# SebLague/Ray-Tracing

Measured on AMD Instinct MI355X. Metric: Mrays/s at 1920x1080, 8 spp, 8 bounces; per-channel L2 vs reference, higher is better.
Workload: dtype f32

## Files before the change

### include/rt_tile_cand.h

```cpp
#ifndef RT_TILE_CAND_ABI_H
#define RT_TILE_CAND_ABI_H

#include "rt_abi.h"

#ifdef __cplusplus
extern "C" {
#endif

int rt_debug_tile_cand(const RtContext* ctx);

#ifdef __cplusplus
}
#endif

#endif
```

### ray-tracing_amd/csrc/rt_context.hip

```cpp
#include <hip/hip_runtime.h>

#include <math.h>
#include <stdarg.h>
#include <stdio.h>
#include <stdlib.h>
#include <string.h>
#include <dlfcn.h>
#include <sys/mman.h>

#include <cmath>
#include <string>
#include <vector>

#include <algorithm>
#include <chrono>
#include <mutex>

#include "rt_kernels.h"
#include "../../include/rt_cost.h"
#include "../../include/rt_primary.h"
#include "../../include/rt_tile_cand.h"
#include "../../include/rt_aov.h"
#include "../../include/rt_denoise.h"
#include "../../include/rt_reproject.h"
// ... 75 lines not shown
    int wavesPerGroup = 1;
    uint32_t hotUnits = 0;
    uint32_t poolSpinLimit = 1u << 16;
    int poolMinItems = 4;
    int poolWaves = 1, poolCells = 0;
    uint32_t travLimit = 1u << 20;
    bool haveScene = false;
    std::vector<RtModel> hModels;
    std::vector<uint32_t> hRootCodes;
    std::vector<int32_t> hTriBase;
    PrimaryTris primaryTris;
    bool primaryOn = true;
    int lastPrimaryOn = -1;
    bool tileCandOn = true;
    int lastTileCand = -1;
    uint32_t* dTileCand[2] = {nullptr, nullptr};
    int tileCandTiles = 0;
    bool tileCandValid[2] = {false, false};
    TileCandKey tileCandKey[2];
    bool tileCandWanted = false;
    TileCandKey tileCandWant;

    RtParams params;
    bool haveParams = false;
    int frame = 1;

    unsigned long long* dCounters = nullptr;
    unsigned long long* dTileQueue = nullptr;
    unsigned long long tileQueueNext[2] = {0, 0};
    uint32_t* dTileCost = nullptr;
// ... 283 lines not shown
        HIP_TRY(ctx, hipStreamSynchronize(ctx->ownStream));
        HIP_TRY(ctx, hipEventCreate(&ctx->evStart));
        HIP_TRY(ctx, hipEventCreate(&ctx->evStop));
        for (hipEvent_t& ev : ctx->backend.ev) HIP_TRY(ctx, hipEventCreateWithFlags(&ev, hipEventDisableTiming));
        return RT_OK;
    };
    if (int rc = init()) {
        rt_destroy(ctx);
        return rc;
    }
    memset(&ctx->params, 0, sizeof(ctx->params));
    if (const char* g = getenv("RT_GRID")) ctx->gridOverride = atoi(g);
    if (const char* g = getenv("RT_POOL_MIN_ITEMS")) ctx->poolMinItems = atoi(g);
    if (const char* g = getenv("RT_PRIMARY")) ctx->primaryOn = atoi(g) != 0;
    if (const char* g = getenv("RT_TILE_CAND")) ctx->tileCandOn = atoi(g) != 0;
    if (const char* g = getenv("RT_POOL_FAULT")) { if (atoi(g)) ctx->poolSpinLimit = 64u | 0x80000000u; }
    if (getenv("RT_VERBOSE")) ctx->verbose = true;
    if (const char* f = getenv("RT_FUSE_FRAMES")) ctx->fuseFrames = atoi(f) != 0;
    if (const char* l = getenv("RT_LPT")) ctx->order.lpt = atoi(l) != 0;
    if (const char* t = getenv("RT_TWO_STREAMS")) ctx->twoStreams = atoi(t) != 0;
    if (const char* c = getenv("RT_COALESCE")) ctx->coalesce = atoi(c) != 0;
    if (const char* fg = getenv("RT_FRAME_GROUP")) ctx->frameGroupOverride = atoi(fg);
    if (const char* al = getenv("RT_ALTERNATE")) ctx->order.alternate = ctx->alternateWanted = atoi(al) != 0;
    ctx->order.set_two_streams(ctx->twoStreams && ctx->sideStream);
    if (const char* fc = getenv("RT_FUSE_CAP"))
        if (const int cap = rt_plan::pinned_fuse_cap(atoi(fc))) { ctx->fuseCap = cap; ctx->fuseCapPinned = true; }
    *out = ctx;
    return RT_OK;
}

// ... 517 lines not shown
        const bool noNegZero = rt_f2u(o.x) != 0x80000000u && rt_f2u(o.y) != 0x80000000u && rt_f2u(o.z) != 0x80000000u;
        a.raygenNoDefocus = (a.defocus == 0.0f && fin && noNegZero && std::isfinite(a.rcpW)) ? 1 : 0;
        const bool allowed = withTable && ctx->haveScene &&
                             primary_allowed(ctx->primaryOn, a.raygenNoDefocus != 0, ctx->flatScene, ctx->nSpheres, ctx->nModels, ctx->primaryTris);
        std::vector<float> sph;
        DModel dm[RT_PRIMARY_MAX_MODELS];
        if (allowed) {
            float bound;
            pack_spheres(ctx->hSpheres.data(), ctx->nSpheres, sph, &bound);
            for (int i = 0; i < ctx->nModels; i++) pack_model(ctx->hModels[i], ctx->hRootCodes[i], ctx->hTriBase[i], dm[i]);
        }
        primary_fill(a.primary, allowed, o, sph.data(), ctx->nSpheres, ctx->sphereBound, dm, ctx->nModels, ctx->primaryTris);
        if (withTable) {
            ctx->lastPrimaryOn = a.primary.on;
            ctx->lastTileCand = 0;
            ctx->tileCandWanted = ctx->tileCandOn && a.primary.on != 0;
            if (ctx->tileCandWanted) {
                TileCandKey& k = ctx->tileCandWant;
                tile_cand_key_init(k);
                memcpy(k.cam, a.cam, sizeof(k.cam));
                memcpy(k.viewParams, a.viewParams, sizeof(k.viewParams));
                k.rcpWm1 = a.rcpWm1; k.rcpHm1 = a.rcpHm1; k.rcpW = a.rcpW; k.diverge = a.diverge;
                k.camOrigin[0] = o.x; k.camOrigin[1] = o.y; k.camOrigin[2] = o.z;
                k.W = (int32_t)a.W; k.H = (int32_t)a.H;
                k.tilesX = a.tilesX; k.tiles = a.tilesX * a.tilesY;
                k.stripRows = a.stripRows; k.partIndex = a.partIndex; k.partCount = a.partCount;
                k.nSpheres = ctx->nSpheres;
                memcpy(k.sph, sph.data(), sizeof(float) * 4 * (size_t)ctx->nSpheres);
            }
        }
    }
    a.counters = ctx->dCounters;
    a.travLimit = ctx->travLimit;
    a.poolSpinLimit = ctx->poolSpinLimit;
    a.wavesPerGroup = 1;
}

}

struct LaunchPlan {
    void (*kern)(const KArgs) = nullptr;
    void (*kernHalf)(const KArgs) = nullptr;
    rt_plan::LaunchShape shape;
// ... 82 lines not shown
    }
    a.tileCost = ctx->dTileCost;
    return RT_OK;
}

static int prepare_tile_cand(RtContext* ctx, int tiles)
{
    if (!ctx->tileCandWanted || ctx->tileCandTiles == tiles) return RT_OK;
    HIP_TRY(ctx, hipStreamSynchronize(joined(ctx)));
    ctx->tileCandTiles = 0;
    for (int s = 0; s < 2; s++) {
        hipFree(ctx->dTileCand[s]); ctx->dTileCand[s] = nullptr;
        ctx->tileCandValid[s] = false;
    }
    for (int s = 0; s < 2; s++)
        if (hipMalloc(&ctx->dTileCand[s], sizeof(uint32_t) * (size_t)tiles) != hipSuccess) {
            (void)hipGetLastError();
            ctx->dTileCand[s] = nullptr;
            ctx->tileCandWanted = false;
            return RT_OK;
        }
    ctx->tileCandTiles = tiles;
    return RT_OK;
}

static_assert(sizeof(float4) == RT_STAGED_PIXEL_BYTES, "a staged colour is one float4");
static int prepare_staging(RtContext* ctx, KArgs& a, int nFrames, size_t nPix, int lane, bool split, bool* unavailable)
{
    *unavailable = false;
    const size_t need = (size_t)nFrames * nPix * RT_STAGED_PIXEL_BYTES;
    if (!ctx->stagingUnavailable && ctx->stagingBytes[lane] < need) {
// ... 159 lines not shown
    hipStream_t st = stream(s);
    a.pxCold = (float4*)((char*)ctx->dPxCold + (size_t)s * ctx->pxColdWaves * RT_COLD_STRIDE_BYTES);
    a.tileQueue = ctx->dTileQueue + s;
    a.tileQueueBase = pp.tileQueueBase;
    a.tileCand = nullptr;
    if (ctx->tileCandWanted && ctx->tileCandTiles == job->tiles && ctx->tileCandWant.tiles == job->tiles) {
        if (!ctx->tileCandValid[s] || memcmp(&ctx->tileCandKey[s], &ctx->tileCandWant, sizeof(TileCandKey)) != 0) {
            ctx->tileCandValid[s] = false;
            hipLaunchKernelGGL(rtk::rt_tile_cand_kernel, dim3((unsigned)((job->tiles + 255) / 256)), dim3(256), 0, st, ctx->tileCandWant, ctx->dTileCand[s]);
            HIP_TRY(ctx, hipGetLastError());
            ctx->tileCandKey[s] = ctx->tileCandWant;
            ctx->tileCandValid[s] = true;
        }
        a.tileCand = ctx->dTileCand[s];
        ctx->lastTileCand = 1;
    }
    RtContext::Tuner::Probe* probe = job->probe;
    const int fuseSlot = nFrames > 1 ? mark_fused_launch_begin(ctx, st) : -1;
    if (probe) hipEventRecord(probe->start, st);
    hipLaunchKernelGGL(parts == 2 ? plan.kernHalf : plan.kern, dim3(pp.grid), dim3(plan.shape.blockThreads), plan.shape.ldsBytes, st, a);
    if (probe) { hipEventRecord(probe->stop, st); probe->live = true; }
    HIP_TRY(ctx, hipGetLastError());
    mark_fused_launch_end(ctx, fuseSlot, st, nFrames);
    ctx->tileQueueNext[s] = pp.queueNext;
    return RT_OK;
}

int HipOrder::accumulate(int s)
{
    int blocks = (int)((job->nPix + 255) / 256);
// ... 291 lines not shown
    if (n > 2 * RT_N_PHASES) out[2 * RT_N_PHASES] = sum_field(h, 6);
    for (int p = 0; p < RT_N_PHASES && 2 * RT_N_PHASES + 1 + p < n; p++) out[2 * RT_N_PHASES + 1 + p] = p < 3 ? sum_field(h, 8 + 2 * RT_N_PHASES + p) : 0;
    return RT_OK;
}

struct DevScratch {
    void* p = nullptr;
    ~DevScratch() { if (p) hipFree(p); }
    hipError_t alloc(size_t bytes) { return hipMalloc(&p, bytes); }
    float* f() const { return (float*)p; }
};

int rt_debug_fused_frames_cap(const RtContext* ctx) { return ctx ? ctx->fuseCap : RT_ERR_INVALID_ARG; }
int rt_debug_primary_table(const RtContext* ctx) { return ctx ? ctx->lastPrimaryOn : RT_ERR_INVALID_ARG; }
int rt_debug_tile_cand(const RtContext* ctx) { return ctx ? ctx->lastTileCand : RT_ERR_INVALID_ARG; }

int rt_debug_intersect(RtContext* ctx, const float* origins, const float* dirs, int n, float* out10)
{
    if (ctx) RT_FLUSH(ctx);
    if (!ctx) return fail(nullptr, RT_ERR_INVALID_ARG, "null context");
    if (!ctx->haveScene) return fail(ctx, RT_ERR_STATE, "rt_debug_intersect before rt_upload_scene");
    if (n < 0 || (n && (!origins || !dirs || !out10))) return fail(ctx, RT_ERR_INVALID_ARG, "rt_debug_intersect: bad arguments");
    if (n == 0) return RT_OK;
    HIP_TRY(ctx, hipSetDevice(ctx->device));
    DevScratch dO, dD, dR;
    HIP_TRY(ctx, dO.alloc((size_t)n * 12));
    HIP_TRY(ctx, dD.alloc((size_t)n * 12));
    HIP_TRY(ctx, dR.alloc((size_t)n * 40));
    HIP_TRY(ctx, hipMemcpy(dO.p, origins, (size_t)n * 12, hipMemcpyHostToDevice));
    HIP_TRY(ctx, hipMemcpy(dD.p, dirs, (size_t)n * 12, hipMemcpyHostToDevice));
// ... 1704 lines not shown
```

### ray-tracing_amd/csrc/rt_kernels.h

```cpp
#ifndef RT_KERNELS_H
#define RT_KERNELS_H

#include <hip/hip_runtime.h>

#include "../../include/rt_abi.h"
#include "../../include/rt_math.h"
#include "rt_device.h"
#include "rt_tile_cand.h"

#ifndef RT_SUSPEND_NUM
#define RT_SUSPEND_NUM 3
#define RT_SUSPEND_DEN 8
#endif
#ifndef RT_INNER_BURST
#define RT_INNER_BURST 3
#endif

namespace rtk {

#define RT_CAS __attribute__((address_space(4)))
#define RT_LDS __attribute__((address_space(3)))

__device__ __forceinline__ float hw_min(float a, float b) { return __builtin_fminf(a, b); }
__device__ __forceinline__ float hw_max(float a, float b) { return __builtin_fmaxf(a, b); }
// ... 145 lines not shown
        bdet = determinant;
    }
}

struct Trav {
    unsigned long long cand;
    int m;
    uint32_t cur;
    int sp;
    bool rootStep;
    rt_f3 lpos, ldir, linv;
    int triBase;
    bool cull;
};

template <bool STATS, bool FLAT, bool MANY, bool ANY = false, bool PRIMARY = false>
__device__ __forceinline__ void begin_intersect(const KArgs& a, rt_f3 rpos, rt_f3 rdir, uint32_t* extBase, SceneHit& h, Trav& t, Stats& st, const float tmax = 0.0f,
                                                const RT_CAS PrimaryTable* pt = nullptr, const uint32_t* tileCand = nullptr, const uint32_t tile = 0u)
{
    h.dst = RT_INF;
    h.obj = -1;
    h.tri = -1;
    h.u = h.v = h.det = 0.0f;
    h.backface = false;

    const RT_CAS float* sph = (const RT_CAS float*)a.spheres;
    const RT_CAS float* sphq = (const RT_CAS float*)a.sphereQuick;
    const float qa = rt_dot(rdir, rdir);
    const float od = __builtin_fmaf(rpos.x, rdir.x, __builtin_fmaf(rpos.y, rdir.y, rpos.z * rdir.z));
    const float oo = PRIMARY ? 0.0f : __builtin_fmaf(rpos.x, rpos.x, __builtin_fmaf(rpos.y, rpos.y, rpos.z * rpos.z));
    const float negMargin = -(7.62939453125e-06f * qa * (PRIMARY ? pt->ooBound : oo + a.sphereBound));
    typedef float rt_f2v __attribute__((ext_vector_type(2)));
    const rt_f2v dx2 = {rdir.x, rdir.x}, dy2 = {rdir.y, rdir.y}, dz2 = {rdir.z, rdir.z};
    const rt_f2v ox2 = {rpos.x, rpos.x}, oy2 = {rpos.y, rpos.y}, oz2 = {rpos.z, rpos.z};
    const rt_f2v od2 = {od, od}, oo2 = {oo, oo}, qa2 = {qa, qa}, m2 = {-2.0f, -2.0f};
    for (int base = 0; base < a.nSpheres; base += 32) {
        const int n = (a.nSpheres - base) < 32 ? (a.nSpheres - base) : 32;
        uint32_t cand = 0;
        if (PRIMARY && tileCand != nullptr) {
            cand = tileCand[tile];
            if (STATS) {
                for (uint32_t rest = ~cand & (n >= 32 ? 0xffffffffu : (1u << n) - 1u); rest; rest &= rest - 1) {
                    const int s = base + __builtin_ctz(rest);
                    const rt_f3 off = rt_v3(pt->sph[s][0], pt->sph[s][1], pt->sph[s][2]);
                    const float qb = 2 * rt_dot(off, rdir);
                    const float disc = qb * qb - 4 * qa * pt->sph[s][3];
                    if (disc >= 0 && (-qb + rt_sqrt(disc)) * rt_rcp(2 * qa) >= 0) st.filterViolations++;
                }
            }
        } else
        for (int k = 0; k < n; k += 2) {
            const RT_CAS float* q = PRIMARY ? &pt->pair[0][0] + 4 * (base + k) : sphq + 4 * (base + k);
            const rt_f2v cx = {q[0], q[1]}, cy = {q[2], q[3]}, cz = {q[4], q[5]}, kk = {q[6], q[7]};
            const rt_f2v cd = __builtin_elementwise_fma(cx, dx2, __builtin_elementwise_fma(cy, dy2, cz * dz2));
            const rt_f2v b = od2 - cd;
            rt_f2v ct = kk;
            if (!PRIMARY) {
                const rt_f2v co = __builtin_elementwise_fma(cx, ox2, __builtin_elementwise_fma(cy, oy2, cz * oz2));
                ct = __builtin_elementwise_fma(m2, co, oo2) + kk;
            }
            const rt_f2v dq = __builtin_elementwise_fma(b, b, -(qa2 * ct));
            const bool keep0 = !(dq.x < negMargin);
            const bool keep1 = (k + 1 < n) && !(dq.y < negMargin);
            if (STATS) {
                for (int j = 0; j < 2 && k + j < n; j++) {
                    const int s = base + k + j;
                    rt_f3 off = rpos - rt_v3(sph[4 * s + 0], sph[4 * s + 1], sph[4 * s + 2]);
                    float qb = 2 * rt_dot(off, rdir);
                    float qc = rt_dot(off, off) - sph[4 * s + 3];
                    float disc = qb * qb - 4 * qa * qc;
                    if (disc >= 0 && !(j ? keep1 : keep0)) st.filterViolations++;
                }
            }
            cand |= ((keep0 ? 1u : 0u) << k) | ((keep1 ? 1u : 0u) << (k + 1));
        }
        if (ANY && h.dst < tmax) cand = 0;
        while (cand) {
            phase_mark<STATS>(st, PH_SPHERE_ROOTS);
            const int k = __builtin_ctz(cand);
            cand &= cand - 1;
            const int s = base + k;
            float4 sp;
            if (PRIMARY) {
                typedef float rt_f4v __attribute__((ext_vector_type(4)));
                const rt_f4v v = *reinterpret_cast<const RT_CAS rt_f4v*>(&pt->sph[s][0]);
                sp = make_float4(v.x, v.y, v.z, v.w);
            }
            else sp = *reinterpret_cast<const float4*>(a.spheres + 4 * s);
            rt_f3 off = PRIMARY ? rt_v3(sp.x, sp.y, sp.z) : rpos - rt_v3(sp.x, sp.y, sp.z);
            float qb = 2 * rt_dot(off, rdir);
            float qc = PRIMARY ? sp.w : rt_dot(off, off) - sp.w;
            float disc = qb * qb - 4 * qa * qc;
            if (!(disc >= 0)) continue;
            float sq = rt_sqrt(disc);
            const float inv2a = rt_rcp(2 * qa);
            float dstNear = rt_max(0.0f, (-qb - sq) * inv2a);
            float dstFar = (-qb + sq) * inv2a;
            if (dstFar >= 0) {
                bool inside = dstNear == 0;
                float d = inside ? dstFar : dstNear;
                if (d < h.dst) {
                    h.dst = d;
                    h.obj = s;
                    h.backface = inside;
                    if (ANY && d < tmax) cand = 0;
                }
            }
        }
    }
    if (STATS) st.sphere += (uint32_t)a.nSpheres;

    unsigned long long cand = 0;
    const RT_CAS DFilter* cf = (const RT_CAS DFilter*)a.filters;
    const int nf = FLAT ? 0 : (MANY ? a.nFiltered : (a.nModels < 64 ? a.nModels : 64));
    if (nf > 0) {
        const rt_f3 winv = rt_v3(__builtin_amdgcn_rcpf(rdir.x), __builtin_amdgcn_rcpf(rdir.y), __builtin_amdgcn_rcpf(rdir.z));
        const bool farOrigin = !(rt_abs(rpos.x) <= a.filterMaxOrigin && rt_abs(rpos.y) <= a.filterMaxOrigin && rt_abs(rpos.z) <= a.filterMaxOrigin);
        auto test_model = [&](int m) -> bool {
            const RT_CAS DFilter& F = cf[m];
            bool keep = true;
// ... 255 lines not shown
                t.cand = 0;
            } else if (t.sp == 0) t.cur = RT_CODE_NEXT_MODEL;
            else t.cur = stackBase[(--t.sp) * RT_WAVE];
        }
        if (++watchdog > a.travLimit) {
            t.cur = RT_CODE_DONE; t.sp = 0; t.cand = 0;
            if ((int)(threadIdx.x & 63) == __ffsll((long long)__ballot(1)) - 1) atomicAdd(a.counters + 7, 1ull);
        }
        RT_TRAV_VOTE();
    } while ((nA + nB + nC) * RT_SUSPEND_DEN > enteredNum);
#undef RT_TRAV_VOTE
    return t.cur == RT_CODE_DONE;
}

template <bool STATS, bool ANY = false, bool PRIMARY = false>
__device__ __forceinline__ void traverse_flat(const KArgs& a, rt_f3 rpos, rt_f3 rdir, SceneHit& h, Stats& st, const float tmax = 0.0f, const RT_CAS PrimaryTable* pt = nullptr)
{
    const RT_CAS DModel* cm = (const RT_CAS DModel*)a.models;
    const DTri* __restrict__ tris = a.tris;
    const RT_CAS float* pr = PRIMARY ? &pt->tri[0][0] : nullptr;
    for (int m = 0; m < a.nModels; m++) {
        if (ANY && __ballot(!(h.dst < tmax)) == 0ull) break;
        const RT_CAS DModel& M = cm[m];
        rt_f3 lpos;
        if (PRIMARY) lpos = rt_v3(pt->lpos[m][0], pt->lpos[m][1], pt->lpos[m][2]);
        else lpos = rt_v3(M.w2l[0] * rpos.x + M.w2l[1] * rpos.y + M.w2l[2] * rpos.z + M.w2l[3] * 1.0f,
                          M.w2l[4] * rpos.x + M.w2l[5] * rpos.y + M.w2l[6] * rpos.z + M.w2l[7] * 1.0f,
                          M.w2l[8] * rpos.x + M.w2l[9] * rpos.y + M.w2l[10] * rpos.z + M.w2l[11] * 1.0f);
        rt_f3 ldir = rt_v3(M.w2l[0] * rdir.x + M.w2l[1] * rdir.y + M.w2l[2] * rdir.z + M.w2l[3] * 0.0f,
                           M.w2l[4] * rdir.x + M.w2l[5] * rdir.y + M.w2l[6] * rdir.z + M.w2l[7] * 0.0f,
                           M.w2l[8] * rdir.x + M.w2l[9] * rdir.y + M.w2l[10] * rdir.z + M.w2l[11] * 0.0f);
        const uint32_t code = M.rootCode;
        uint32_t count = (code >> 24) & 0x7fu;
        uint32_t start = code & RT_CODE_MAX_INLINE_START;
        if (count == 0) {
            count = a.bigLeaves[2 * start + 1];
            start = a.bigLeaves[2 * start];
        }
        if (STATS) { st.leaf++; st.tri += count; }
        const int first = M.triBase + (int)start;
        const bool cull = M.cullBackface != 0;
        for (uint32_t i = 0; i < count; i++) {
            phase_mark<STATS>(st, PH_TRI);
            if (ANY && h.dst < tmax) break;
            const float before = h.dst;
            tri_test<PRIMARY>(tris, first + 3 * (int)i, lpos, ldir, cull, h.dst, h.tri, h.u, h.v, h.det, pr);
            if (PRIMARY) pr += 4;
            if (h.dst < before) {
                h.obj = a.nSpheres + m;
                h.backface = h.det < 0;
            }
        }
    }
}

template <bool STATS>
__device__ __forceinline__ void intersect_scene(const KArgs& a, rt_f3 rpos, rt_f3 rdir, uint32_t* stackBase, uint32_t* extBase, SceneHit& h, Stats& st)
{
    Trav t;
    if (a.nChunks) {
        begin_intersect<STATS, false, true>(a, rpos, rdir, extBase, h, t, st);
        traverse<STATS, false, true>(a, rpos, rdir, stackBase, extBase, h, t, st, (const RT_LDS char*)nullptr, 0u);
    } else {
        begin_intersect<STATS, false, false>(a, rpos, rdir, extBase, h, t, st);
        traverse<STATS, false, false>(a, rpos, rdir, stackBase, extBase, h, t, st, (const RT_LDS char*)nullptr, 0u);
    }
}
// ... 391 lines not shown
                    if constexpr (COST) if (pathActive) {
                        uint4* const o = RT_COST_SLOT(c) + 1;
                        uint4 p = *o;
                        p.x -= st.inner; p.y -= st.leaf; p.z -= st.tri;
                        *o = p;
                    }
                }
            }
            if (pathActive) {
                phase_mark<STATS>(st, PH_SPHERES);
                if constexpr (FLAT && !MANY && !COST) {
                    const RT_CAS PrimaryTable* const pt = &cold_args().primary;
                    if (pt->on != 0 && __ballot(bounce != 0) == 0ull) {
                        const uint32_t* const tileCand = cold_args().tileCand;
                        const uint32_t tile = tileCand ? __float_as_uint(PX_COLD(cold_args())[RT_WAVE].w) : 0u;
                        begin_intersect<STATS, FLAT, MANY, false, true>(a, rpos, rdir, extBase, h, t, st, 0.0f, pt, tileCand, tile);
                        traverse_flat<STATS, false, true>(a, rpos, rdir, h, st, 0.0f, pt);
                    } else {
                        begin_intersect<STATS, FLAT, MANY>(a, rpos, rdir, extBase, h, t, st);
                        traverse_flat<STATS>(a, rpos, rdir, h, st);
                    }
                    segments++;
                    inTrav = true;
                } else {
                    begin_intersect<STATS, FLAT, MANY>(a, rpos, rdir, extBase, h, t, st);
                    segments++;
                    inTrav = true;
                    if (FLAT) traverse_flat<STATS>(a, rpos, rdir, h, st);
                }
            }
        }
        if constexpr (!POOL) {
// ... 347 lines not shown
    __syncthreads();
    if (t == 0) {
        uint32_t run = 0;
        for (int k = 0; k < 1024; k++) { base[k] = run; run += hist[k]; }
    }
    __syncthreads();
    for (int i = t; i < nTiles; i += 1024) order[atomicAdd(&base[key[i]], 1u)] = (uint32_t)i;
}

__global__ void __launch_bounds__(256) rt_tile_cand_kernel(const TileCandKey k, uint32_t* out)
{
    const int tile = (int)(blockIdx.x * 256u + threadIdx.x);
    if (tile >= k.tiles) return;
    int x0, y0;
    tile_cand_origin(k, tile, &x0, &y0);
    out[tile] = tile_cand_mask(k, x0, y0);
}

__global__ void rt_display_kernel(const float4* src, float4* dst, size_t n, int frame)
{
    const float inv = rt_rcp((float)frame);
    size_t i = (size_t)blockIdx.x * blockDim.x + threadIdx.x;
    const size_t stride = (size_t)gridDim.x * blockDim.x;
    for (; i < n; i += stride) {
        float4 v = src[i];
        dst[i] = make_float4(v.x * inv, v.y * inv, v.z * inv, v.w * inv);
    }
}
__global__ void rt_display_srgb8_kernel(const float4* src, uint32_t* dst, int width, int rows, int frame, int flipY)
{
    const float inv = rt_rcp((float)frame);
// ... 53 lines not shown
```

### ray-tracing_amd/csrc/rt_primary.h

```cpp
#ifndef RT_PRIMARY_H
#define RT_PRIMARY_H

#include <math.h>
#include <stdint.h>
#include <string.h>

#include <cmath>

#include "../../include/rt_math.h"
#include "rt_records.h"

#define RT_PRIMARY_MAX_SPHERES 32
#define RT_PRIMARY_MAX_MODELS 4
#define RT_PRIMARY_MAX_TRIS 16

struct alignas(16) PrimaryTable {
    int32_t on;
    float ooBound;
    int32_t pad[2];
    float camOrigin[4];
    float lpos[RT_PRIMARY_MAX_MODELS][4];
    float pair[RT_PRIMARY_MAX_SPHERES / 2][8];
    float sph[RT_PRIMARY_MAX_SPHERES][4];
    float tri[RT_PRIMARY_MAX_TRIS][4];
};

struct PrimaryTris {
    bool usable = false;
    int nModels = 0;
    int count[RT_PRIMARY_MAX_MODELS] = {0, 0, 0, 0};
    float a[RT_PRIMARY_MAX_TRIS][3];
    float face[RT_PRIMARY_MAX_TRIS][3];
};

static inline void primary_collect_tris(bool flat, const DModel* models, int nModels, const unsigned char* triSpace, size_t triSpaceBytes,
                                        const uint32_t* bigLeaves, size_t nBigLeafWords, PrimaryTris& out)
{
    out = PrimaryTris();
    if (!flat || nModels < 0 || nModels > RT_PRIMARY_MAX_MODELS) return;
    int total = 0;
    for (int m = 0; m < nModels; m++) {
        const uint32_t code = models[m].rootCode;
        uint32_t count = (code >> 24) & 0x7fu, start = code & RT_CODE_MAX_INLINE_START;
        if (count == 0) {
            if (2 * (size_t)start + 1 >= nBigLeafWords) return;
            count = bigLeaves[2 * (size_t)start + 1];
            start = bigLeaves[2 * (size_t)start];
        }
        if (count > (uint32_t)(RT_PRIMARY_MAX_TRIS - total)) return;
        for (uint32_t i = 0; i < count; i++) {
            const long long unit = (long long)models[m].triBase + (long long)start + 3ll * (long long)i;
            if (unit < 0 || ((size_t)unit + 3) * 16 > triSpaceBytes) return;
            DTri t;
            memcpy(&t, triSpace + (size_t)unit * 16, sizeof(t));
            out.a[total][0] = t.ax; out.a[total][1] = t.ay; out.a[total][2] = t.az;
            out.face[total][0] = t.fx; out.face[total][1] = t.fy; out.face[total][2] = t.fz;
            total++;
        }
        out.count[m] = (int)count;
    }
    out.nModels = nModels;
    out.usable = true;
}

static inline bool primary_allowed(bool switchOn, bool noDefocus, bool flatScene, int nSpheres, int nModels, const PrimaryTris& tris)
{
    return switchOn && noDefocus && flatScene && nSpheres >= 0 && nSpheres <= RT_PRIMARY_MAX_SPHERES && nModels >= 0 && nModels <= RT_PRIMARY_MAX_MODELS &&
           tris.usable && tris.nModels == nModels;
}

static inline rt_f3 primary_cam_origin(const float* cam) { return rt_mul_point(cam, rt_v3(0.0f, 0.0f, 0.0f), 1.0f); }
// ... 50 lines not shown
```

### ray-tracing_amd/csrc/rt_tile_cand.h

```cpp
#ifndef RT_TILE_CAND_H
#define RT_TILE_CAND_H

#include <stdint.h>
#include <string.h>

#include "../../include/rt_math.h"

#define RT_TILE_CAND_MAX_SPHERES 32

struct TileCandKey {
    float cam[16];
    float viewParams[3];
    float rcpWm1, rcpHm1, rcpW, diverge;
    float camOrigin[3];
    int32_t W, H;
    int32_t tilesX, tiles;
    int32_t stripRows, partIndex, partCount;
    int32_t nSpheres;
    float sph[RT_TILE_CAND_MAX_SPHERES][4];
};

static inline void tile_cand_key_init(TileCandKey& k) { memset(&k, 0, sizeof(k)); }

RT_HD void tile_cand_origin(const TileCandKey& k, int tile, int* x0, int* y0)
{
    const int ty = tile / k.tilesX;
    const int row0 = ty * 8;
    const int ls = row0 / k.stripRows;
    *x0 = (tile - ty * k.tilesX) * 8;
    *y0 = (ls * k.partCount + k.partIndex) * k.stripRows + (row0 - ls * k.stripRows);
}

RT_HD bool tile_cand_finite(float x) { return rt_abs(x) < RT_INF; }

// ... 25 lines not shown
        const float re = slack * rt_sqrt(rr + 7.62939453125e-06f * (D2 + rr)) + scale;
        const float sa2 = slack * slack * (Rt * Rt) / L2, sb2 = slack * slack * (re * re) / D2;
        const rt_f3 cr = rt_cross(a, v);
        const float cross2 = rt_dot(cr, cr), av = rt_dot(a, v);
        const float lim = L2 * D2;
        bool drop = false;
        if (tile_cand_finite(sa2) && tile_cand_finite(sb2) && tile_cand_finite(cross2) && tile_cand_finite(av) && tile_cand_finite(lim) && sa2 + sb2 < 0.98f) {
            const float sg = rt_sqrt(sa2) * rt_sqrt(1.0f - sb2) + rt_sqrt(1.0f - sa2) * rt_sqrt(sb2);
            drop = (av <= 0.0f) || (cross2 > sg * sg * lim);
        }
        if (!drop) mask |= 1u << s;
    }
    return mask;
}

#endif
```

### ray-tracing_amd/hip.py

```python
import ctypes as C
import os

import numpy as np

from . import abi

_HERE = os.path.dirname(os.path.abspath(__file__))
LIB_PATH = os.environ.get("RT_HIP_LIB") or os.path.join(_HERE, "lib", "libraytrace_hip.so")

ABI_SYMBOLS = [
    "rt_create", "rt_destroy", "rt_last_error", "rt_set_stream", "rt_resize", "rt_set_partition", "rt_local_rows",
    "rt_local_to_global_row", "rt_bind_render_targets", "rt_get_render_targets", "rt_upload_scene", "rt_update_models",
    "rt_update_spheres", "rt_set_params", "rt_reset_accumulation", "rt_render_frame", "rt_render_frames",
    "rt_synchronize", "rt_get_frame", "rt_read_frame", "rt_read_accumulated", "rt_display", "rt_display_srgb8",
    "rt_write_accumulated", "rt_timer_begin", "rt_timer_end",
    "rt_enable_stats", "rt_reset_counters", "rt_get_counters", "rt_build_bvh", "rt_build_bvh_mt", "rt_build_bvh_gpu", "rt_build_bvh_gpu_release", "rt_camera_view_params", "rt_version",
    "rt_debug_intersect", "rt_debug_math_eval", "rt_debug_phase_profile", "rt_build_bvh_gpu_batch",
    "rt_flush", "rt_validate_scene", "rt_debug_layout", "rt_debug_layout_free", "rt_debug_fused_frames_cap",
    "rt_create_multi", "rt_destroy_multi", "rt_multi_count", "rt_multi_context", "rt_multi_resize", "rt_multi_upload_scene",
    "rt_multi_update_models", "rt_multi_update_spheres", "rt_multi_set_params", "rt_multi_reset_accumulation",
    "rt_multi_render_frame", "rt_multi_render_frames", "rt_multi_synchronize", "rt_gather_accumulated", "rt_gather_frame",
    "rt_multi_get_counters", "rt_multi_last_gather_ms", "rt_multi_peer_access", "rt_gather_accumulated_to_device", "rt_gather_frame_to_device",
    "rt_gather_rccl",
]
COST_SYMBOLS = ["rt_render_cost"]
PRIMARY_SYMBOLS = ["rt_debug_primary_table"]
TILE_CAND_SYMBOLS = ["rt_debug_tile_cand"]
AOV_SYMBOLS = ["rt_render_aov", "rt_render_aov_to_device"]
DENOISE_SYMBOLS = ["rt_denoise_default_params", "rt_denoise_buffers", "rt_denoise", "rt_denoise_to_device"]
REPROJECT_SYMBOLS = ["rt_reproject_default_params", "rt_reproject_buffers", "rt_reproject_accumulated", "rt_resolve_buffers", "rt_resolve",
                     "rt_resolve_to_device"]
MOTION_SYMBOLS = ["rt_render_aov_centre", "rt_render_aov_centre_to_device", "rt_motion_from_scene", "rt_reproject_buffers_moving",
                  "rt_reproject_accumulated_moving"]
VARIANCE_SYMBOLS = ["rt_denoise_variance_default_params", "rt_moments_update_buffers", "rt_denoise_variance_buffers", "rt_variance_update",
                    "rt_variance_reset", "rt_variance_carry", "rt_variance_read_moments", "rt_variance_moments_to_device", "rt_denoise_variance",
                    "rt_denoise_variance_to_device"]
ADAPTIVE_SYMBOLS = ["rt_adaptive_default_params", "rt_adaptive_select_buffers", "rt_adaptive_select", "rt_adaptive_set_tiles", "rt_adaptive_read_tiles",
                    "rt_adaptive_read_tile_error", "rt_adaptive_render_frames"]
QUERY_SYMBOLS = ["rt_query_closest", "rt_query_closest_buffers", "rt_query_occluded", "rt_query_occluded_buffers"]
RADIANCE_SYMBOLS = ["rt_radiance_trace", "rt_radiance_trace_buffers"]
COST_FIELDS = ("segments", "innerSteps", "leafSteps", "triTests", "primaryInnerSteps", "primaryLeafSteps", "primaryTriTests", "firstHit")

# ... 434 lines not shown
        self._check(self.api.gather_rccl(self.h, nccl_comm, int(root), 1 if accumulated else 0, device_ptr, nbytes))

    def fused_frames_cap(self):
        return self.api.debug_fused_frames_cap(self.h)

    def primary_table(self):
        fn = self.api.lib.rt_debug_primary_table
        fn.restype, fn.argtypes = C.c_int, [C.c_void_p]
        return fn(self.h)

    def tile_cand(self):
        fn = self.api.lib.rt_debug_tile_cand
        fn.restype, fn.argtypes = C.c_int, [C.c_void_p]
        return fn(self.h)

    def synchronize(self):
        self._check(self.api.synchronize(self.h))

    def flush(self):
        self._check(self.api.flush(self.h))

    def timer_begin(self):
        self._check(self.api.timer_begin(self.h))

    def timer_end(self):
        self._check(self.api.timer_end(self.h))

    def enable_stats(self, on=True):
        self._check(self.api.enable_stats(self.h, 1 if on else 0))

# ... 205 lines not shown
```

Baseline: 52920.

## Add per-tile triangle candidate masks to cull primary-ray triangle tests

Extends the per-tile candidate precompute to triangles in flat primary tables. A conservative frustum-versus-triangle-wedge test builds a bitmask per tile, and the wave-wide union of these masks gates which triangles traverse_flat tests for primary rays. When no lane needs any triangle, the flat traversal is skipped entirely. The sphere candidate path is also split out so it no longer runs the 32-sphere base loop. The cost is a doubled candidate buffer, a larger key, ballot/readlane loops, and the risk of wrongly culling a triangle if the conservative bounds are off.

```diff
diff --git a/include/rt_tile_cand.h b/include/rt_tile_cand.h
--- a/include/rt_tile_cand.h
+++ b/include/rt_tile_cand.h
@@ -2,6 +2,7 @@
 #define RT_TILE_CAND_ABI_H
 
 #include "rt_abi.h"
+#include "rt_tile_tri.h"
 
 #ifdef __cplusplus
 extern "C" {
diff --git a/include/rt_tile_tri.h b/include/rt_tile_tri.h
--- /dev/null
+++ b/include/rt_tile_tri.h
@@ -0,0 +1,16 @@
+#ifndef RT_TILE_TRI_ABI_H
+#define RT_TILE_TRI_ABI_H
+
+#include "rt_abi.h"
+
+#ifdef __cplusplus
+extern "C" {
+#endif
+
+int rt_debug_tile_tri(const RtContext* ctx);
+
+#ifdef __cplusplus
+}
+#endif
+
+#endif
diff --git a/ray-tracing_amd/csrc/rt_context.hip b/ray-tracing_amd/csrc/rt_context.hip
--- a/ray-tracing_amd/csrc/rt_context.hip
+++ b/ray-tracing_amd/csrc/rt_context.hip
@@ -113,6 +113,8 @@
     int lastPrimaryOn = -1;
     bool tileCandOn = true;
     int lastTileCand = -1;
+    bool tileTriOn = true;
+    int lastTileTri = -1;
     uint32_t* dTileCand[2] = {nullptr, nullptr};
     int tileCandTiles = 0;
     bool tileCandValid[2] = {false, false};
@@ -426,6 +428,7 @@
     if (const char* g = getenv("RT_POOL_MIN_ITEMS")) ctx->poolMinItems = atoi(g);
     if (const char* g = getenv("RT_PRIMARY")) ctx->primaryOn = atoi(g) != 0;
     if (const char* g = getenv("RT_TILE_CAND")) ctx->tileCandOn = atoi(g) != 0;
+    if (const char* g = getenv("RT_TILE_TRI")) ctx->tileTriOn = atoi(g) != 0;
     if (const char* g = getenv("RT_POOL_FAULT")) { if (atoi(g)) ctx->poolSpinLimit = 64u | 0x80000000u; }
     if (getenv("RT_VERBOSE")) ctx->verbose = true;
     if (const char* f = getenv("RT_FUSE_FRAMES")) ctx->fuseFrames = atoi(f) != 0;
@@ -973,6 +976,7 @@
         if (withTable) {
             ctx->lastPrimaryOn = a.primary.on;
             ctx->lastTileCand = 0;
+            ctx->lastTileTri = 0;
             ctx->tileCandWanted = ctx->tileCandOn && a.primary.on != 0;
             if (ctx->tileCandWanted) {
                 TileCandKey& k = ctx->tileCandWant;
@@ -986,6 +990,21 @@
                 k.stripRows = a.stripRows; k.partIndex = a.partIndex; k.partCount = a.partCount;
                 k.nSpheres = ctx->nSpheres;
                 memcpy(k.sph, sph.data(), sizeof(float) * 4 * (size_t)ctx->nSpheres);
+                const PrimaryTris& pt = ctx->primaryTris;
+                k.triOn = ctx->tileTriOn ? 1 : 0;
+                if (k.triOn) {
+                    k.nTriModels = ctx->nModels;
+                    int t = 0;
+                    for (int m = 0; m < ctx->nModels; m++) {
+                        k.triCount[m] = pt.count[m];
+                        memcpy(k.w2l[m], dm[m].w2l, sizeof(k.w2l[m]));
+                        memcpy(k.lpos[m], a.primary.lpos[m], sizeof(k.lpos[m]));
+                        for (int i = 0; i < pt.count[m]; i++, t++) {
+                            memcpy(&k.tri[t][0], pt.a[t], 12); memcpy(&k.tri[t][3], pt.ab[t], 12);
+                            memcpy(&k.tri[t][6], pt.ac[t], 12); memcpy(&k.tri[t][9], pt.face[t], 12);
+                        }
+                    }
+                }
             }
         }
     }
@@ -1098,7 +1117,7 @@
         ctx->tileCandValid[s] = false;
     }
     for (int s = 0; s < 2; s++)
-        if (hipMalloc(&ctx->dTileCand[s], sizeof(uint32_t) * (size_t)tiles) != hipSuccess) {
+        if (hipMalloc(&ctx->dTileCand[s], 2 * sizeof(uint32_t) * (size_t)tiles) != hipSuccess) {
             (void)hipGetLastError();
             ctx->dTileCand[s] = nullptr;
             ctx->tileCandWanted = false;
@@ -1288,6 +1307,7 @@
         }
         a.tileCand = ctx->dTileCand[s];
         ctx->lastTileCand = 1;
+        ctx->lastTileTri = ctx->tileCandWant.triOn;
     }
     RtContext::Tuner::Probe* probe = job->probe;
     const int fuseSlot = nFrames > 1 ? mark_fused_launch_begin(ctx, st) : -1;
@@ -1609,6 +1629,7 @@
 int rt_debug_fused_frames_cap(const RtContext* ctx) { return ctx ? ctx->fuseCap : RT_ERR_INVALID_ARG; }
 int rt_debug_primary_table(const RtContext* ctx) { return ctx ? ctx->lastPrimaryOn : RT_ERR_INVALID_ARG; }
 int rt_debug_tile_cand(const RtContext* ctx) { return ctx ? ctx->lastTileCand : RT_ERR_INVALID_ARG; }
+int rt_debug_tile_tri(const RtContext* ctx) { return ctx ? ctx->lastTileTri : RT_ERR_INVALID_ARG; }
 
 int rt_debug_intersect(RtContext* ctx, const float* origins, const float* dirs, int n, float* out10)
 {
diff --git a/ray-tracing_amd/csrc/rt_kernels.h b/ray-tracing_amd/csrc/rt_kernels.h
--- a/ray-tracing_amd/csrc/rt_kernels.h
+++ b/ray-tracing_amd/csrc/rt_kernels.h
@@ -183,9 +183,14 @@
     bool cull;
 };
 
+struct TriWant {
+    uint32_t wave;
+    uint32_t lane;
+};
 template <bool STATS, bool FLAT, bool MANY, bool ANY = false, bool PRIMARY = false>
 __device__ __forceinline__ void begin_intersect(const KArgs& a, rt_f3 rpos, rt_f3 rdir, uint32_t* extBase, SceneHit& h, Trav& t, Stats& st, const float tmax = 0.0f,
-                                                const RT_CAS PrimaryTable* pt = nullptr, const uint32_t* tileCand = nullptr, const uint32_t tile = 0u)
+                                                const RT_CAS PrimaryTable* pt = nullptr, const uint32_t* tileCand = nullptr, const uint32_t tile = 0u,
+                                                TriWant* tw = nullptr)
 {
     h.dst = RT_INF;
     h.obj = -1;
@@ -193,86 +198,123 @@
     h.u = h.v = h.det = 0.0f;
     h.backface = false;
 
-    const RT_CAS float* sph = (const RT_CAS float*)a.spheres;
-    const RT_CAS float* sphq = (const RT_CAS float*)a.sphereQuick;
-    const float qa = rt_dot(rdir, rdir);
-    const float od = __builtin_fmaf(rpos.x, rdir.x, __builtin_fmaf(rpos.y, rdir.y, rpos.z * rdir.z));
-    const float oo = PRIMARY ? 0.0f : __builtin_fmaf(rpos.x, rpos.x, __builtin_fmaf(rpos.y, rpos.y, rpos.z * rpos.z));
-    const float negMargin = -(7.62939453125e-06f * qa * (PRIMARY ? pt->ooBound : oo + a.sphereBound));
-    typedef float rt_f2v __attribute__((ext_vector_type(2)));
-    const rt_f2v dx2 = {rdir.x, rdir.x}, dy2 = {rdir.y, rdir.y}, dz2 = {rdir.z, rdir.z};
-    const rt_f2v ox2 = {rpos.x, rpos.x}, oy2 = {rpos.y, rpos.y}, oz2 = {rpos.z, rpos.z};
-    const rt_f2v od2 = {od, od}, oo2 = {oo, oo}, qa2 = {qa, qa}, m2 = {-2.0f, -2.0f};
-    for (int base = 0; base < a.nSpheres; base += 32) {
-        const int n = (a.nSpheres - base) < 32 ? (a.nSpheres - base) : 32;
-        uint32_t cand = 0;
-        if (PRIMARY && tileCand != nullptr) {
-            cand = tileCand[tile];
-            if (STATS) {
-                for (uint32_t rest = ~cand & (n >= 32 ? 0xffffffffu : (1u << n) - 1u); rest; rest &= rest - 1) {
-                    const int s = base + __builtin_ctz(rest);
-                    const rt_f3 off = rt_v3(pt->sph[s][0], pt->sph[s][1], pt->sph[s][2]);
-                    const float qb = 2 * rt_dot(off, rdir);
-                    const float disc = qb * qb - 4 * qa * pt->sph[s][3];
-                    if (disc >= 0 && (-qb + rt_sqrt(disc)) * rt_rcp(2 * qa) >= 0) st.filterViolations++;
-                }
-            }
-        } else
-        for (int k = 0; k < n; k += 2) {
-            const RT_CAS float* q = PRIMARY ? &pt->pair[0][0] + 4 * (base + k) : sphq + 4 * (base + k);
-            const rt_f2v cx = {q[0], q[1]}, cy = {q[2], q[3]}, cz = {q[4], q[5]}, kk = {q[6], q[7]};
-            const rt_f2v cd = __builtin_elementwise_fma(cx, dx2, __builtin_elementwise_fma(cy, dy2, cz * dz2));
-            const rt_f2v b = od2 - cd;
-            rt_f2v ct = kk;
-            if (!PRIMARY) {
-                const rt_f2v co = __builtin_elementwise_fma(cx, ox2, __builtin_elementwise_fma(cy, oy2, cz * oz2));
-                ct = __builtin_elementwise_fma(m2, co, oo2) + kk;
-            }
-            const rt_f2v dq = __builtin_elementwise_fma(b, b, -(qa2 * ct));
-            const bool keep0 = !(dq.x < negMargin);
-            const bool keep1 = (k + 1 < n) && !(dq.y < negMargin);
-            if (STATS) {
-                for (int j = 0; j < 2 && k + j < n; j++) {
-                    const int s = base + k + j;
-                    rt_f3 off = rpos - rt_v3(sph[4 * s + 0], sph[4 * s + 1], sph[4 * s + 2]);
-                    float qb = 2 * rt_dot(off, rdir);
-                    float qc = rt_dot(off, off) - sph[4 * s + 3];
-                    float disc = qb * qb - 4 * qa * qc;
-                    if (disc >= 0 && !(j ? keep1 : keep0)) st.filterViolations++;
-                }
-            }
-            cand |= ((keep0 ? 1u : 0u) << k) | ((keep1 ? 1u : 0u) << (k + 1));
-        }
-        if (ANY && h.dst < tmax) cand = 0;
-        while (cand) {
-            phase_mark<STATS>(st, PH_SPHERE_ROOTS);
-            const int k = __builtin_ctz(cand);
-            cand &= cand - 1;
-            const int s = base + k;
-            float4 sp;
-            if (PRIMARY) {
+    if (PRIMARY && tileCand != nullptr) {
+        const uint2 entry = reinterpret_cast<const uint2*>(tileCand)[tile];
+        uint32_t cand = entry.x;
+        if (tw != nullptr) {
+            uint32_t want = 0u;
+            for (unsigned long long more = __ballot(entry.y != 0u); more != 0ull; more = __ballot((entry.y & ~want) != 0u))
+                want |= (uint32_t)__builtin_amdgcn_readlane((int)entry.y, __builtin_ctzll(more));
+            tw->wave = want;
+            if (STATS) tw->lane = entry.y;
+        }
+        if (STATS) {
+            const float qa = rt_dot(rdir, rdir);
+            for (uint32_t rest = ~cand & (a.nSpheres >= 32 ? 0xffffffffu : (1u << a.nSpheres) - 1u); rest; rest &= rest - 1) {
+                const int s = __builtin_ctz(rest);
+                const rt_f3 off = rt_v3(pt->sph[s][0], pt->sph[s][1], pt->sph[s][2]);
+                const float qb = 2 * rt_dot(off, rdir);
+                const float disc = qb * qb - 4 * qa * pt->sph[s][3];
+                if (disc >= 0 && (-qb + rt_sqrt(disc)) * rt_rcp(2 * qa) >= 0) st.filterViolations++;
+            }
+        }
+        if (cand != 0u) {
+            const float qa = rt_dot(rdir, rdir);
+            const float inv2a = rt_rcp(2 * qa);
+            do {
+                phase_mark<STATS>(st, PH_SPHERE_ROOTS);
+                const int s = __builtin_ctz(cand);
+                cand &= cand - 1;
                 typedef float rt_f4v __attribute__((ext_vector_type(4)));
-                const rt_f4v v = *reinterpret_cast<const RT_CAS rt_f4v*>(&pt->sph[s][0]);
-                sp = make_float4(v.x, v.y, v.z, v.w);
-            }
-            else sp = *reinterpret_cast<const float4*>(a.spheres + 4 * s);
-            rt_f3 off = PRIMARY ? rt_v3(sp.x, sp.y, sp.z) : rpos - rt_v3(sp.x, sp.y, sp.z);
-            float qb = 2 * rt_dot(off, rdir);
-            float qc = PRIMARY ? sp.w : rt_dot(off, off) - sp.w;
-            float disc = qb * qb - 4 * qa * qc;
-            if (!(disc >= 0)) continue;
-            float sq = rt_sqrt(disc);
-            const float inv2a = rt_rcp(2 * qa);
-            float dstNear = rt_max(0.0f, (-qb - sq) * inv2a);
-            float dstFar = (-qb + sq) * inv2a;
-            if (dstFar >= 0) {
-                bool inside = dstNear == 0;
-                float d = inside ? dstFar : dstNear;
-                if (d < h.dst) {
-                    h.dst = d;
-                    h.obj = s;
-                    h.backface = inside;
-                    if (ANY && d < tmax) cand = 0;
+                const rt_f4v sp = *reinterpret_cast<const RT_CAS rt_f4v*>(&pt->sph[s][0]);
+                const rt_f3 off = rt_v3(sp.x, sp.y, sp.z);
+                const float qb = 2 * rt_dot(off, rdir);
+                const float disc = qb * qb - 4 * qa * sp.w;
+                if (!(disc >= 0)) continue;
+                const float sq = rt_sqrt(disc);
+                const float dstNear = rt_max(0.0f, (-qb - sq) * inv2a);
+                const float dstFar = (-qb + sq) * inv2a;
+                if (dstFar >= 0) {
+                    const bool inside = dstNear == 0;
+                    const float d = inside ? dstFar : dstNear;
+                    if (d < h.dst) {
+                        h.dst = d;
+                        h.obj = s;
+                        h.backface = inside;
+                    }
+                }
+            } while (cand != 0u);
+        }
+    } else {
+        const RT_CAS float* sph = (const RT_CAS float*)a.spheres;
+        const RT_CAS float* sphq = (const RT_CAS float*)a.sphereQuick;
+        const float qa = rt_dot(rdir, rdir);
+        const float od = __builtin_fmaf(rpos.x, rdir.x, __builtin_fmaf(rpos.y, rdir.y, rpos.z * rdir.z));
+        const float oo = PRIMARY ? 0.0f : __builtin_fmaf(rpos.x, rpos.x, __builtin_fmaf(rpos.y, rpos.y, rpos.z * rpos.z));
+        const float negMargin = -(7.62939453125e-06f * qa * (PRIMARY ? pt->ooBound : oo + a.sphereBound));
+        typedef float rt_f2v __attribute__((ext_vector_type(2)));
+        const rt_f2v dx2 = {rdir.x, rdir.x}, dy2 = {rdir.y, rdir.y}, dz2 = {rdir.z, rdir.z};
+        const rt_f2v ox2 = {rpos.x, rpos.x}, oy2 = {rpos.y, rpos.y}, oz2 = {rpos.z, rpos.z};
+        const rt_f2v od2 = {od, od}, oo2 = {oo, oo}, qa2 = {qa, qa}, m2 = {-2.0f, -2.0f};
+        for (int base = 0; base < a.nSpheres; base += 32) {
+            const int n = (a.nSpheres - base) < 32 ? (a.nSpheres - base) : 32;
+            uint32_t cand = 0;
+            for (int k = 0; k < n; k += 2) {
+                const RT_CAS float* q = PRIMARY ? &pt->pair[0][0] + 4 * (base + k) : sphq + 4 * (base + k);
+                const rt_f2v cx = {q[0], q[1]}, cy = {q[2], q[3]}, cz = {q[4], q[5]}, kk = {q[6], q[7]};
+                const rt_f2v cd = __builtin_elementwise_fma(cx, dx2, __builtin_elementwise_fma(cy, dy2, cz * dz2));
+                const rt_f2v b = od2 - cd;
+                rt_f2v ct = kk;
+                if (!PRIMARY) {
+                    const rt_f2v co = __builtin_elementwise_fma(cx, ox2, __builtin_elementwise_fma(cy, oy2, cz * oz2));
+                    ct = __builtin_elementwise_fma(m2, co, oo2) + kk;
+                }
+                const rt_f2v dq = __builtin_elementwise_fma(b, b, -(qa2 * ct));
+                const bool keep0 = !(dq.x < negMargin);
+                const bool keep1 = (k + 1 < n) && !(dq.y < negMargin);
+                if (STATS) {
+                    for (int j = 0; j < 2 && k + j < n; j++) {
+                        const int s = base + k + j;
+                        rt_f3 off = rpos - rt_v3(sph[4 * s + 0], sph[4 * s + 1], sph[4 * s + 2]);
+                        float qb = 2 * rt_dot(off, rdir);
+                        float qc = rt_dot(off, off) - sph[4 * s + 3];
+                        float disc = qb * qb - 4 * qa * qc;
+                        if (disc >= 0 && !(j ? keep1 : keep0)) st.filterViolations++;
+                    }
+                }
+                cand |= ((keep0 ? 1u : 0u) << k) | ((keep1 ? 1u : 0u) << (k + 1));
+            }
+            if (ANY && h.dst < tmax) cand = 0;
+            while (cand) {
+                phase_mark<STATS>(st, PH_SPHERE_ROOTS);
+                const int k = __builtin_ctz(cand);
+                cand &= cand - 1;
+                const int s = base + k;
+                float4 sp;
+                if (PRIMARY) {
+                    typedef float rt_f4v __attribute__((ext_vector_type(4)));
+                    const rt_f4v v = *reinterpret_cast<const RT_CAS rt_f4v*>(&pt->sph[s][0]);
+                    sp = make_float4(v.x, v.y, v.z, v.w);
+                }
+                else sp = *reinterpret_cast<const float4*>(a.spheres + 4 * s);
+                rt_f3 off = PRIMARY ? rt_v3(sp.x, sp.y, sp.z) : rpos - rt_v3(sp.x, sp.y, sp.z);
+                float qb = 2 * rt_dot(off, rdir);
+                float qc = PRIMARY ? sp.w : rt_dot(off, off) - sp.w;
+                float disc = qb * qb - 4 * qa * qc;
+                if (!(disc >= 0)) continue;
+                float sq = rt_sqrt(disc);
+                const float inv2a = rt_rcp(2 * qa);
+                float dstNear = rt_max(0.0f, (-qb - sq) * inv2a);
+                float dstFar = (-qb + sq) * inv2a;
+                if (dstFar >= 0) {
+                    bool inside = dstNear == 0;
+                    float d = inside ? dstFar : dstNear;
+                    if (d < h.dst) {
+                        h.dst = d;
+                        h.obj = s;
+                        h.backface = inside;
+                        if (ANY && d < tmax) cand = 0;
+                    }
                 }
             }
         }
@@ -558,11 +600,13 @@
 }
 
 template <bool STATS, bool ANY = false, bool PRIMARY = false>
-__device__ __forceinline__ void traverse_flat(const KArgs& a, rt_f3 rpos, rt_f3 rdir, SceneHit& h, Stats& st, const float tmax = 0.0f, const RT_CAS PrimaryTable* pt = nullptr)
+__device__ __forceinline__ void traverse_flat(const KArgs& a, rt_f3 rpos, rt_f3 rdir, SceneHit& h, Stats& st, const float tmax = 0.0f, const RT_CAS PrimaryTable* pt = nullptr,
+                                              const uint32_t triWant = 0xffffffffu, const uint32_t triLane = 0xffffffffu)
 {
     const RT_CAS DModel* cm = (const RT_CAS DModel*)a.models;
     const DTri* __restrict__ tris = a.tris;
     const RT_CAS float* pr = PRIMARY ? &pt->tri[0][0] : nullptr;
+    uint32_t tk = 0u;
     for (int m = 0; m < a.nModels; m++) {
         if (ANY && __ballot(!(h.dst < tmax)) == 0ull) break;
         const RT_CAS DModel& M = cm[m];
@@ -571,9 +615,13 @@
         else lpos = rt_v3(M.w2l[0] * rpos.x + M.w2l[1] * rpos.y + M.w2l[2] * rpos.z + M.w2l[3] * 1.0f,
                           M.w2l[4] * rpos.x + M.w2l[5] * rpos.y + M.w2l[6] * rpos.z + M.w2l[7] * 1.0f,
                           M.w2l[8] * rpos.x + M.w2l[9] * rpos.y + M.w2l[10] * rpos.z + M.w2l[11] * 1.0f);
-        rt_f3 ldir = rt_v3(M.w2l[0] * rdir.x + M.w2l[1] * rdir.y + M.w2l[2] * rdir.z + M.w2l[3] * 0.0f,
-                           M.w2l[4] * rdir.x + M.w2l[5] * rdir.y + M.w2l[6] * rdir.z + M.w2l[7] * 0.0f,
-                           M.w2l[8] * rdir.x + M.w2l[9] * rdir.y + M.w2l[10] * rdir.z + M.w2l[11] * 0.0f);
+        auto local_dir = [&]() {
+            return rt_v3(M.w2l[0] * rdir.x + M.w2l[1] * rdir.y + M.w2l[2] * rdir.z + M.w2l[3] * 0.0f,
+                         M.w2l[4] * rdir.x + M.w2l[5] * rdir.y + M.w2l[6] * rdir.z + M.w2l[7] * 0.0f,
+                         M.w2l[8] * rdir.x + M.w2l[9] * rdir.y + M.w2l[10] * rdir.z + M.w2l[11] * 0.0f);
+        };
+        rt_f3 ldir;
+        if (!PRIMARY) ldir = local_dir();
         const uint32_t code = M.rootCode;
         uint32_t count = (code >> 24) & 0x7fu;
         uint32_t start = code & RT_CODE_MAX_INLINE_START;
@@ -582,9 +630,31 @@
             start = a.bigLeaves[2 * start];
         }
         if (STATS) { st.leaf++; st.tri += count; }
+        uint32_t wantM = 0xffffffffu;
+        if (PRIMARY) {
+            wantM = (triWant >> tk) & ((1u << count) - 1u);
+            if (!STATS && wantM == 0u) {
+                tk += count;
+                pr += 4 * count;
+                continue;
+            }
+            ldir = local_dir();
+        }
         const int first = M.triBase + (int)start;
         const bool cull = M.cullBackface != 0;
         for (uint32_t i = 0; i < count; i++) {
+            if (PRIMARY) {
+                if (STATS && !((triLane >> (tk + i)) & 1u)) {
+                    float best = RT_INF, bu, bv, bdet;
+                    int btri = -1;
+                    tri_test<PRIMARY>(tris, first + 3 * (int)i, lpos, ldir, cull, best, btri, bu, bv, bdet, pr);
+                    if (btri >= 0) st.filterViolations++;
+                }
+                if (!((wantM >> i) & 1u)) {
+                    pr += 4;
+                    continue;
+                }
+            }
             phase_mark<STATS>(st, PH_TRI);
             if (ANY && h.dst < tmax) break;
             const float before = h.dst;
@@ -595,6 +665,7 @@
                 h.backface = h.det < 0;
             }
         }
+        if (PRIMARY) tk += count;
     }
 }
 
@@ -1016,8 +1087,10 @@
                     if (pt->on != 0 && __ballot(bounce != 0) == 0ull) {
                         const uint32_t* const tileCand = cold_args().tileCand;
                         const uint32_t tile = tileCand ? __float_as_uint(PX_COLD(cold_args())[RT_WAVE].w) : 0u;
-                        begin_intersect<STATS, FLAT, MANY, false, true>(a, rpos, rdir, extBase, h, t, st, 0.0f, pt, tileCand, tile);
-                        traverse_flat<STATS, false, true>(a, rpos, rdir, h, st, 0.0f, pt);
+                        TriWant tw = {0xffffffffu, 0xffffffffu};
+                        begin_intersect<STATS, FLAT, MANY, false, true>(a, rpos, rdir, extBase, h, t, st, 0.0f, pt, tileCand, tile, &tw);
+                        if (STATS || tw.wave != 0u)
+                            traverse_flat<STATS, false, true>(a, rpos, rdir, h, st, 0.0f, pt, tw.wave, tw.lane);
                     } else {
                         begin_intersect<STATS, FLAT, MANY>(a, rpos, rdir, extBase, h, t, st);
                         traverse_flat<STATS>(a, rpos, rdir, h, st);
@@ -1395,7 +1468,8 @@
     if (tile >= k.tiles) return;
     int x0, y0;
     tile_cand_origin(k, tile, &x0, &y0);
-    out[tile] = tile_cand_mask(k, x0, y0);
+    out[2 * tile] = tile_cand_mask(k, x0, y0);
+    out[2 * tile + 1] = k.triOn ? tile_tri_mask(k, x0, y0) : 0xffffffffu;
 }
 
 __global__ void rt_display_kernel(const float4* src, float4* dst, size_t n, int frame)
diff --git a/ray-tracing_amd/csrc/rt_primary.h b/ray-tracing_amd/csrc/rt_primary.h
--- a/ray-tracing_amd/csrc/rt_primary.h
+++ b/ray-tracing_amd/csrc/rt_primary.h
@@ -31,6 +31,8 @@
     int count[RT_PRIMARY_MAX_MODELS] = {0, 0, 0, 0};
     float a[RT_PRIMARY_MAX_TRIS][3];
     float face[RT_PRIMARY_MAX_TRIS][3];
+    float ab[RT_PRIMARY_MAX_TRIS][3];
+    float ac[RT_PRIMARY_MAX_TRIS][3];
 };
 
 static inline void primary_collect_tris(bool flat, const DModel* models, int nModels, const unsigned char* triSpace, size_t triSpaceBytes,
@@ -55,6 +57,8 @@
             memcpy(&t, triSpace + (size_t)unit * 16, sizeof(t));
             out.a[total][0] = t.ax; out.a[total][1] = t.ay; out.a[total][2] = t.az;
             out.face[total][0] = t.fx; out.face[total][1] = t.fy; out.face[total][2] = t.fz;
+            out.ab[total][0] = t.abx; out.ab[total][1] = t.aby; out.ab[total][2] = t.abz;
+            out.ac[total][0] = t.acx; out.ac[total][1] = t.acy; out.ac[total][2] = t.acz;
             total++;
         }
         out.count[m] = (int)count;
diff --git a/ray-tracing_amd/csrc/rt_tile_cand.h b/ray-tracing_amd/csrc/rt_tile_cand.h
--- a/ray-tracing_amd/csrc/rt_tile_cand.h
+++ b/ray-tracing_amd/csrc/rt_tile_cand.h
@@ -7,6 +7,8 @@
 #include "../../include/rt_math.h"
 
 #define RT_TILE_CAND_MAX_SPHERES 32
+#define RT_TILE_TRI_MAX_MODELS 4
+#define RT_TILE_TRI_MAX_TRIS 16
 
 struct TileCandKey {
     float cam[16];
@@ -18,6 +20,12 @@
     int32_t stripRows, partIndex, partCount;
     int32_t nSpheres;
     float sph[RT_TILE_CAND_MAX_SPHERES][4];
+    int32_t triOn;
+    int32_t nTriModels;
+    int32_t triCount[RT_TILE_TRI_MAX_MODELS];
+    float w2l[RT_TILE_TRI_MAX_MODELS][12];
+    float lpos[RT_TILE_TRI_MAX_MODELS][4];
+    float tri[RT_TILE_TRI_MAX_TRIS][12];
 };
 
 static inline void tile_cand_key_init(TileCandKey& k) { memset(&k, 0, sizeof(k)); }
@@ -73,4 +81,75 @@
     return mask;
 }
 
+RT_HD uint32_t tile_tri_mask(const TileCandKey& k, int x0, int y0)
+{
+    const int nm = k.nTriModels < RT_TILE_TRI_MAX_MODELS ? k.nTriModels : RT_TILE_TRI_MAX_MODELS;
+    int n = 0;
+    for (int m = 0; m < nm; m++) n += k.triCount[m] > 0 ? k.triCount[m] : 0;
+    if (n > RT_TILE_TRI_MAX_TRIS) n = RT_TILE_TRI_MAX_TRIS;
+    const uint32_t all = (1u << n) - 1u;
+    if (k.W <= 1 || k.H <= 1) return all;
+    const float eps = 6.103515625e-05f;
+    const float lo = 1.52587890625e-05f, hi = 65536.0f;
+    const rt_f3 o = rt_v3(k.camOrigin[0], k.camOrigin[1], k.camOrigin[2]);
+    const rt_f3 R = rt_v3(k.cam[0], k.cam[1], k.cam[2]), U = rt_v3(k.cam[4], k.cam[5], k.cam[6]), F = rt_v3(k.cam[8], k.cam[9], k.cam[10]);
+    const float fx = (((float)x0 + 3.5f) * k.rcpWm1 - 0.5f) * k.viewParams[0];
+    const float fy = (((float)y0 + 3.5f) * k.rcpHm1 - 0.5f) * k.viewParams[1];
+    const float jit = 1.01f * rt_abs(k.diverge * k.rcpW);
+    const float ex = 4.0f * rt_abs(k.rcpWm1 * k.viewParams[0]) + jit, ey = 4.0f * rt_abs(k.rcpHm1 * k.viewParams[1]) + jit;
+    rt_f3 g[4];
+    float gmax = 0.0f;
+    for (int j = 0; j < 4; j++) {
+        g[j] = F * k.viewParams[2] + R * ((j & 1) ? fx + ex : fx - ex) + U * ((j & 2) ? fy + ey : fy - ey);
+        const float len = rt_sqrt(rt_dot(g[j], g[j]));
+        if (!tile_cand_finite(len)) return all;
+        gmax = rt_max(gmax, len);
+    }
+    const float lenO = rt_sqrt(rt_dot(o, o));
+    if (!(tile_cand_finite(lenO) && lenO <= hi && gmax >= lo && gmax <= hi)) return all;
+    uint32_t mask = 0;
+    int t = 0;
+    for (int m = 0; m < nm; m++) {
+        const float* w = k.w2l[m];
+        const float wn = rt_abs(w[0]) + rt_abs(w[1]) + rt_abs(w[2]) + rt_abs(w[4]) + rt_abs(w[5]) + rt_abs(w[6]) + rt_abs(w[8]) + rt_abs(w[9]) + rt_abs(w[10]);
+        rt_f3 c[4];
+        for (int j = 0; j < 4; j++)
+            c[j] = rt_v3(w[0] * g[j].x + w[1] * g[j].y + w[2] * g[j].z, w[4] * g[j].x + w[5] * g[j].y + w[6] * g[j].z, w[8] * g[j].x + w[9] * g[j].y + w[10] * g[j].z);
+        const float dirScale = wn * (lenO + gmax);
+        const rt_f3 lpos = rt_v3(k.lpos[m][0], k.lpos[m][1], k.lpos[m][2]);
+        const float lenL = rt_sqrt(rt_dot(lpos, lpos));
+        const bool modelOk = wn >= lo && wn <= hi && tile_cand_finite(lenL);
+        for (int i = 0; i < k.triCount[m] && t < n; i++, t++) {
+            const float* q = k.tri[t];
+            const rt_f3 A = rt_v3(q[0], q[1], q[2]), AB = rt_v3(q[3], q[4], q[5]), AC = rt_v3(q[6], q[7], q[8]), face = rt_v3(q[9], q[10], q[11]);
+            const rt_f3 p = lpos - A;
+            const float e = rt_dot(p, face);
+            const float lenP = lenL + rt_sqrt(rt_dot(A, A));
+            const float nab = rt_sqrt(rt_dot(AB, AB)), nac = rt_sqrt(rt_dot(AC, AC)), nf = rt_sqrt(rt_dot(face, face));
+            const float NU = lenP * nac, NV = lenP * nab, ND = nf, NW = ND + NU + NV;
+            bool drop = false;
+            if (modelOk && lenP >= lo && lenP <= hi && nab >= lo && nab <= hi && nac >= lo && nac <= hi && nf >= lo * lo && nf <= hi * hi &&
+                tile_cand_finite(e) && rt_abs(e) > eps * lenP * nf) {
+                const float s = e > 0.0f ? 1.0f : -1.0f;
+                const rt_f3 nD = face * (-s), nU = rt_cross(AC, p) * s, nV = rt_cross(p, AB) * s, nW = nD - nU - nV;
+                const rt_f3 nrm[4] = {nD, nU, nV, nW};
+                const float bound[4] = {ND, NU, NV, NW};
+                bool sound = true;
+                for (int f = 0; f < 4; f++) {
+                    const float l2 = rt_dot(nrm[f], nrm[f]), z = eps * bound[f];
+                    sound = sound && tile_cand_finite(l2) && l2 > z * z;
+                }
+                for (int f = 0; f < 4 && sound && !drop; f++) {
+                    const float margin = eps * bound[f] * dirScale;
+                    bool out = tile_cand_finite(margin);
+                    for (int j = 0; j < 4; j++) out = out && rt_dot(nrm[f], c[j]) < -margin;
+                    drop = out;
+                }
+            }
+            if (!drop) mask |= 1u << t;
+        }
+    }
+    return mask | (all & ~((t >= 32 ? 0u : (1u << t)) - 1u));
+}
+
 #endif
diff --git a/ray-tracing_amd/hip.py b/ray-tracing_amd/hip.py
--- a/ray-tracing_amd/hip.py
+++ b/ray-tracing_amd/hip.py
@@ -26,6 +26,7 @@
 COST_SYMBOLS = ["rt_render_cost"]
 PRIMARY_SYMBOLS = ["rt_debug_primary_table"]
 TILE_CAND_SYMBOLS = ["rt_debug_tile_cand"]
+TILE_TRI_SYMBOLS = ["rt_debug_tile_tri"]
 AOV_SYMBOLS = ["rt_render_aov", "rt_render_aov_to_device"]
 DENOISE_SYMBOLS = ["rt_denoise_default_params", "rt_denoise_buffers", "rt_denoise", "rt_denoise_to_device"]
 REPROJECT_SYMBOLS = ["rt_reproject_default_params", "rt_reproject_buffers", "rt_reproject_accumulated", "rt_resolve_buffers", "rt_resolve",
@@ -490,6 +491,11 @@
         fn.restype, fn.argtypes = C.c_int, [C.c_void_p]
         return fn(self.h)
 
+    def tile_tri(self):
+        fn = self.api.lib.rt_debug_tile_tri
+        fn.restype, fn.argtypes = C.c_int, [C.c_void_p]
+        return fn(self.h)
+
     def synchronize(self):
         self._check(self.api.synchronize(self.h))
 
```

Measured after the change: 54670, median of 6. 3.3% higher.
